# spacemeshos/go-spacemesh

Hardware: AMD Instinct MI355X
Metric: post_labels_per_sec (higher is better)
Workload: dtype u32; 1 GPU; init-mainnet-scryptN8192-4units-256GiB-sink; step_labels=2097152, scrypt_n=8192, num_units=4, labels_per_unit=4294967296, parallelism=index-range shards x1, RCCL nonce min-reduce, vrf_nonce_found=True

## Files before the change

go-spacemesh_amd/csrc/kernel_args.h:

```cpp
#ifndef POST_KERNEL_ARGS_H
#define POST_KERNEL_ARGS_H

#include <hip/hip_runtime.h>

#include "post_common.h"

struct LabelKernelArgs {
  uint32_t commitment_le[8];
  uint64_t start;
  uint64_t count;
  uint32_t scrypt_n;
  uint32_t gap_shift;
  uint32_t out_full;
  uint32_t *scratch;
  uint64_t scratch_lanes;
  uint8_t *out;
  const uint64_t *indices;
  const uint32_t *commit_ids;
  const uint32_t *commitments;
  uint32_t *xbuf;
  uint32_t has_difficulty;
  uint32_t difficulty_be[8];
  PostVrfCandidate *cand;
  unsigned int *cand_count;
  uint32_t cand_cap;
};

struct ScanKernelArgs {
  const uint4 *labels;
  uint64_t count;
  uint64_t index_base;
  const uint32_t *te;
  const uint8_t *sbox;
  const uint32_t *rk;
  uint32_t n_ciphers;
  uint64_t difficulty;
  PostScanHit *hits;
  unsigned int *hit_count;
  uint32_t hit_cap;
};

struct VerifyPredArgs {
  const uint4 *labels2;
  uint64_t count;
  const uint32_t *te;
  const uint8_t *sbox;
  const uint32_t *rk;
  const uint32_t *task_proof;
  const uint8_t *half;
  const uint64_t *difficulty;
  uint8_t *pass;
};

extern "C" {
hipError_t poste_launch_label_kernel(const LabelKernelArgs *args,
                                     uint32_t blocks, hipStream_t stream);
hipError_t poste_launch_verify_pred_kernel(const VerifyPredArgs *args,
                                           uint32_t blocks,
                                           hipStream_t stream);
hipError_t poste_launch_scan_kernel(const ScanKernelArgs *args,
                                    uint32_t blocks, hipStream_t stream);
uint64_t poste_label_resident_slots(uint32_t gap_shift);
}

#endif
```

go-spacemesh_amd/csrc/kernels.hip:

```cpp
#include <hip/hip_runtime.h>

#include <cstdlib>
#include <cstring>

#include "kernel_args.h"
#include "post_common.h"

#define POSTE_THREADS 256

#if defined(POSTE_NT) && POSTE_NT
typedef uint32_t poste_v4u __attribute__((ext_vector_type(4)));
#define VSTORE(p, v)                                                           \
  do {                                                                         \
    uint4 _t = (v);                                                            \
    __builtin_nontemporal_store(*(poste_v4u *)&_t, (poste_v4u *)(p));          \
  } while (0)
#define VLOAD(p)                                                               \
  ({                                                                           \
    poste_v4u _r = __builtin_nontemporal_load((const poste_v4u *)(p));         \
    *(uint4 *)&_r;                                                             \
  })
#else
#define VSTORE(p, v) (*(p) = (v))
#define VLOAD(p) (*(p))
#endif

__constant__ uint32_t c_sha_k[64] = {
    0x428a2f98, 0x71374491, 0xb5c0fbcf, 0xe9b5dba5, 0x3956c25b, 0x59f111f1,
    0x923f82a4, 0xab1c5ed5, 0xd807aa98, 0x12835b01, 0x243185be, 0x550c7dc3,
    0x72be5d74, 0x80deb1fe, 0x9bdc06a7, 0xc19bf174, 0xe49b69c1, 0xefbe4786,
    0x0fc19dc6, 0x240ca1cc, 0x2de92c6f, 0x4a7484aa, 0x5cb0a9dc, 0x76f988da,
    0x983e5152, 0xa831c66d, 0xb00327c8, 0xbf597fc7, 0xc6e00bf3, 0xd5a79147,
    0x06ca6351, 0x14292967, 0x27b70a85, 0x2e1b2138, 0x4d2c6dfc, 0x53380d13,
    0x650a7354, 0x766a0abb, 0x81c2c92e, 0x92722c85, 0xa2bfe8a1, 0xa81a664b,
    0xc24b8b70, 0xc76c51a3, 0xd192e819, 0xd6990624, 0xf40e3585, 0x106aa070,
    0x19a4c116, 0x1e376c08, 0x2748774c, 0x34b0bcb5, 0x391c0cb3, 0x4ed8aa4a,
    0x5b9cca4f, 0x682e6ff3, 0x748f82ee, 0x78a5636f, 0x84c87814, 0x8cc70208,
    0x90befffa, 0xa4506ceb, 0xbef9a3f7, 0xc67178f2};

__device__ __forceinline__ uint32_t ror32(uint32_t x, int n) {
  return __builtin_rotateright32(x, n);
}

__device__ void sha_compress(uint32_t h[8], const uint32_t m[16]) {
  uint32_t w[16];
#pragma unroll
  for (int i = 0; i < 16; i++) w[i] = m[i];
  uint32_t a = h[0], b = h[1], c = h[2], d = h[3];
  uint32_t e = h[4], f = h[5], g = h[6], hh = h[7];
#pragma unroll
  for (int t = 0; t < 64; t++) {
    uint32_t wt;
    if (t < 16) {
      wt = w[t];
    } else {
      uint32_t a15 = w[(t - 15) & 15], a2 = w[(t - 2) & 15];
      wt = w[t & 15] += (ror32(a15, 7) ^ ror32(a15, 18) ^ (a15 >> 3)) +
                        w[(t - 7) & 15] +
                        (ror32(a2, 17) ^ ror32(a2, 19) ^ (a2 >> 10));
    }
    uint32_t t1 = hh + (ror32(e, 6) ^ ror32(e, 11) ^ ror32(e, 25)) +
                  ((e & f) ^ (~e & g)) + c_sha_k[t] + wt;
    uint32_t t2 = (ror32(a, 2) ^ ror32(a, 13) ^ ror32(a, 22)) +
                  ((a & b) ^ (a & c) ^ (b & c));
    hh = g; g = f; f = e; e = d + t1;
    d = c; c = b; b = a; a = t1 + t2;
  }
  h[0] += a; h[1] += b; h[2] += c; h[3] += d;
  h[4] += e; h[5] += f; h[6] += g; h[7] += hh;
}

__device__ __forceinline__ void sha_init(uint32_t h[8]) {
  h[0] = 0x6a09e667; h[1] = 0xbb67ae85; h[2] = 0x3c6ef372; h[3] = 0xa54ff53a;
  h[4] = 0x510e527f; h[5] = 0x9b05688c; h[6] = 0x1f83d9ab; h[7] = 0x5be0cd19;
}


#define SWZ(v, pat)                                                            \
  ((uint32_t)__builtin_amdgcn_mov_dpp((int)(v), (pat), 0xf, 0xf, true))
#define QROT1 0x39
#define QROT2 0x4E
#define QROT3 0x93
#define QBCAST0 0x00

__device__ __forceinline__ void salsa8_z(uint32_t &A, uint32_t &B,
                                         uint32_t &C, uint32_t &D) {
  uint32_t a = A, b = B, c = C, d = D;
#pragma unroll
  for (int i = 0; i < 4; i++) {
    b ^= __builtin_rotateleft32(a + d, 7);
    c ^= __builtin_rotateleft32(b + a, 9);
    d ^= __builtin_rotateleft32(c + b, 13);
    a ^= __builtin_rotateleft32(d + c, 18);
    uint32_t y1 = SWZ(d, QROT1);
    uint32_t y2 = SWZ(c, QROT2);
    uint32_t y3 = SWZ(b, QROT3);
    y1 ^= __builtin_rotateleft32(a + y3, 7);
    y2 ^= __builtin_rotateleft32(y1 + a, 9);
    y3 ^= __builtin_rotateleft32(y2 + y1, 13);
    a ^= __builtin_rotateleft32(y3 + y2, 18);
    d = SWZ(y1, QROT3);
    c = SWZ(y2, QROT2);
    b = SWZ(y3, QROT1);
  }
  A += a; B += b; C += c; D += d;
}

__device__ __forceinline__ void salsa8_z2(uint32_t &A0, uint32_t &B0,
                                          uint32_t &C0, uint32_t &D0,
                                          uint32_t &A1, uint32_t &B1,
                                          uint32_t &C1, uint32_t &D1) {
  uint32_t a0 = A0, b0 = B0, c0 = C0, d0 = D0;
  uint32_t a1 = A1, b1 = B1, c1 = C1, d1 = D1;
#pragma unroll
  for (int i = 0; i < 4; i++) {
    b0 ^= __builtin_rotateleft32(a0 + d0, 7);
    b1 ^= __builtin_rotateleft32(a1 + d1, 7);
    c0 ^= __builtin_rotateleft32(b0 + a0, 9);
    c1 ^= __builtin_rotateleft32(b1 + a1, 9);
    d0 ^= __builtin_rotateleft32(c0 + b0, 13);
    d1 ^= __builtin_rotateleft32(c1 + b1, 13);
    a0 ^= __builtin_rotateleft32(d0 + c0, 18);
    a1 ^= __builtin_rotateleft32(d1 + c1, 18);
    uint32_t y30 = SWZ(b0, QROT3), y31 = SWZ(b1, QROT3);
    uint32_t y20 = SWZ(c0, QROT2), y21 = SWZ(c1, QROT2);
    uint32_t y10 = SWZ(d0, QROT1), y11 = SWZ(d1, QROT1);
    y10 ^= __builtin_rotateleft32(a0 + y30, 7);
    y11 ^= __builtin_rotateleft32(a1 + y31, 7);
    y20 ^= __builtin_rotateleft32(y10 + a0, 9);
    y21 ^= __builtin_rotateleft32(y11 + a1, 9);
    y30 ^= __builtin_rotateleft32(y20 + y10, 13);
    y31 ^= __builtin_rotateleft32(y21 + y11, 13);
    a0 ^= __builtin_rotateleft32(y30 + y20, 18);
    a1 ^= __builtin_rotateleft32(y31 + y21, 18);
    d0 = SWZ(y10, QROT3);
    d1 = SWZ(y11, QROT3);
    c0 = SWZ(y20, QROT2);
    c1 = SWZ(y21, QROT2);
    b0 = SWZ(y30, QROT1);
    b1 = SWZ(y31, QROT1);
  }
  A0 += a0; B0 += b0; C0 += c0; D0 += d0;
  A1 += a1; B1 += b1; C1 += c1; D1 += d1;
}

__device__ __forceinline__ void blockmix2_z(uint32_t XA0[4], uint32_t XA1[4],
                                            uint32_t XB0[4],
                                            uint32_t XB1[4]) {
  uint32_t ta0 = XA0[0] ^ XA1[0], ta1 = XA0[1] ^ XA1[1],
           ta2 = XA0[2] ^ XA1[2], ta3 = XA0[3] ^ XA1[3];
  uint32_t tb0 = XB0[0] ^ XB1[0], tb1 = XB0[1] ^ XB1[1],
           tb2 = XB0[2] ^ XB1[2], tb3 = XB0[3] ^ XB1[3];
  salsa8_z2(ta0, ta1, ta2, ta3, tb0, tb1, tb2, tb3);
  XA0[0] = ta0; XA0[1] = ta1; XA0[2] = ta2; XA0[3] = ta3;
  XB0[0] = tb0; XB0[1] = tb1; XB0[2] = tb2; XB0[3] = tb3;
  ta0 ^= XA1[0]; ta1 ^= XA1[1]; ta2 ^= XA1[2]; ta3 ^= XA1[3];
  tb0 ^= XB1[0]; tb1 ^= XB1[1]; tb2 ^= XB1[2]; tb3 ^= XB1[3];
  salsa8_z2(ta0, ta1, ta2, ta3, tb0, tb1, tb2, tb3);
  XA1[0] = ta0; XA1[1] = ta1; XA1[2] = ta2; XA1[3] = ta3;
  XB1[0] = tb0; XB1[1] = tb1; XB1[2] = tb2; XB1[3] = tb3;
}

__device__ __forceinline__ void blockmix_z(uint32_t X0[4], uint32_t X1[4]) {
  uint32_t t0 = X0[0] ^ X1[0], t1 = X0[1] ^ X1[1], t2 = X0[2] ^ X1[2],
           t3 = X0[3] ^ X1[3];
  salsa8_z(t0, t1, t2, t3);
  X0[0] = t0; X0[1] = t1; X0[2] = t2; X0[3] = t3;
  t0 ^= X1[0]; t1 ^= X1[1]; t2 ^= X1[2]; t3 ^= X1[3];
  salsa8_z(t0, t1, t2, t3);
  X1[0] = t0; X1[1] = t1; X1[2] = t2; X1[3] = t3;
}

__device__ __forceinline__ void canon_to_z(const uint32_t x[16], uint32_t sub,
                                           uint32_t z[4]) {
  uint32_t s0 = sub == 0 ? x[0] : sub == 1 ? x[5] : sub == 2 ? x[10] : x[15];
  uint32_t s1 = sub == 0 ? x[4] : sub == 1 ? x[9] : sub == 2 ? x[14] : x[3];
  uint32_t s2 = sub == 0 ? x[8] : sub == 1 ? x[13] : sub == 2 ? x[2] : x[7];
  uint32_t s3 = sub == 0 ? x[12] : sub == 1 ? x[1] : sub == 2 ? x[6] : x[11];
  z[0] = s0; z[1] = s1; z[2] = s2; z[3] = s3;
}

__device__ __forceinline__ void z_to_msg_be(const uint32_t z[4],
                                            uint32_t m[16]) {
#pragma unroll
  for (int v = 0; v < 4; v++) {
    m[(4 * v + 0) & 15] = __builtin_bswap32(SWZ(z[v], 0x00));
    m[(4 * v + 5) & 15] = __builtin_bswap32(SWZ(z[v], 0x55));
    m[(4 * v + 10) & 15] = __builtin_bswap32(SWZ(z[v], 0xAA));
    m[(4 * v + 15) & 15] = __builtin_bswap32(SWZ(z[v], 0xFF));
  }
}


__device__ __forceinline__ void hmac_outer(const uint32_t ho[8],
                                           const uint32_t inner[8],
                                           uint32_t out[8]) {
  uint32_t h[8], m[16];
#pragma unroll
  for (int i = 0; i < 8; i++) h[i] = ho[i];
#pragma unroll
  for (int i = 0; i < 8; i++) m[i] = inner[i];
  m[8] = 0x80000000u;
#pragma unroll
  for (int i = 9; i < 15; i++) m[i] = 0;
  m[15] = (64 + 32) * 8;
  sha_compress(h, m);
#pragma unroll
  for (int i = 0; i < 8; i++) out[i] = h[i];
}


__device__ __forceinline__ void hmac_states_for(const uint32_t *cw,
                                                unsigned long long index,
                                                uint32_t hi[8],
                                                uint32_t ho[8]) {
  uint32_t pw_be[10], m[16];
#pragma unroll
  for (int i = 0; i < 8; i++) pw_be[i] = __builtin_bswap32(cw[i]);
  pw_be[8] = __builtin_bswap32((uint32_t)index);
  pw_be[9] = __builtin_bswap32((uint32_t)(index >> 32));
  sha_init(hi);
#pragma unroll
  for (int i = 0; i < 10; i++) m[i] = pw_be[i] ^ 0x36363636u;
#pragma unroll
  for (int i = 10; i < 16; i++) m[i] = 0x36363636u;
  sha_compress(hi, m);
  sha_init(ho);
#pragma unroll
  for (int i = 0; i < 10; i++) m[i] = pw_be[i] ^ 0x5c5c5c5cu;
#pragma unroll
  for (int i = 10; i < 16; i++) m[i] = 0x5c5c5c5cu;
  sha_compress(ho, m);
}

__global__ void __launch_bounds__(POSTE_THREADS)
post_label_prologue_kernel(LabelKernelArgs a) {
  const unsigned long long lane =
      (unsigned long long)blockIdx.x * blockDim.x + threadIdx.x;
  const unsigned long long group = lane >> 2;
  const unsigned long long gstride =
      ((unsigned long long)gridDim.x * blockDim.x) >> 2;
  const uint32_t sub = (uint32_t)(lane & 3);
  uint4 *X = (uint4 *)a.xbuf;

  for (unsigned long long task = group; task < a.count;
       task += gstride) {
    const unsigned long long index = a.indices ? a.indices[task]
                                               : a.start + task;
    const uint32_t *cw = a.commit_ids
                             ? a.commitments + 8ull * a.commit_ids[task]
                             : a.commitment_le;
    uint32_t hi[8], ho[8], m[16];
    hmac_states_for(cw, index, hi, ho);
    uint32_t Z0[4], Z1[4];
    for (uint32_t half = 0; half < 2; half++) {
      uint32_t cblk[16];
#pragma unroll
      for (uint32_t q = 0; q < 2; q++) {
        const uint32_t blk = half * 2 + q + 1;
        uint32_t h[8];
#pragma unroll
        for (int i = 0; i < 8; i++) h[i] = hi[i];
        m[0] = blk;
        m[1] = 0x80000000u;
#pragma unroll
        for (int i = 2; i < 15; i++) m[i] = 0;
        m[15] = (64 + 4) * 8;
        sha_compress(h, m);
        uint32_t d[8];
        hmac_outer(ho, h, d);
#pragma unroll
        for (int k = 0; k < 8; k++)
          cblk[8 * q + k] = __builtin_bswap32(d[k]);
      }
      canon_to_z(cblk, sub, half == 0 ? Z0 : Z1);
    }
    uint4 *p = X + task * 8ull;
    p[sub] = make_uint4(Z0[0], Z0[1], Z0[2], Z0[3]);
    p[sub + 4] = make_uint4(Z1[0], Z1[1], Z1[2], Z1[3]);
  }
}

__global__ void __launch_bounds__(POSTE_THREADS, 8)
post_label_romix_kernel(LabelKernelArgs a) {
  const unsigned long long lane =
      (unsigned long long)blockIdx.x * blockDim.x + threadIdx.x;
  const unsigned long long group = lane >> 2;
  const uint32_t sub = (uint32_t)(lane & 3);
  const uint32_t n = a.scrypt_n;
  const uint32_t mask = n - 1;
  const uint32_t gmask = (1u << a.gap_shift) - 1u;
  uint4 *V = (uint4 *)a.scratch;
  uint4 *X = (uint4 *)a.xbuf;

  for (unsigned long long task = group; task < a.count;
       task += a.scratch_lanes) {
    uint32_t Z0[4], Z1[4];
    {
      uint4 *p = X + task * 8ull;
      uint4 v0 = p[sub], v1 = p[sub + 4];
      Z0[0] = v0.x; Z0[1] = v0.y; Z0[2] = v0.z; Z0[3] = v0.w;
      Z1[0] = v1.x; Z1[1] = v1.y; Z1[2] = v1.z; Z1[3] = v1.w;
    }
    {
      unsigned long long base = group * 8ull + sub;
      const unsigned long long stride = a.scratch_lanes * 8ull;
      for (uint32_t j = 0; j < n; j++) {
        if ((j & gmask) == 0) {
          uint4 *p = V + base;
          VSTORE(p, make_uint4(Z0[0], Z0[1], Z0[2], Z0[3]));
          VSTORE(p + 4, make_uint4(Z1[0], Z1[1], Z1[2], Z1[3]));
          base += stride;
        }
        blockmix_z(Z0, Z1);
      }
    }
    for (uint32_t i = 0; i < n; i++) {
      uint32_t j = SWZ(Z1[0], QBCAST0) & mask;
      const uint32_t r = j & gmask;
      const uint4 *p =
          V + ((unsigned long long)(j >> a.gap_shift) * a.scratch_lanes +
               group) * 8ull + sub;
      uint32_t Y0[4], Y1[4];
      {
        uint4 v0 = VLOAD(p), v1 = VLOAD(p + 4);
        Y0[0] = v0.x; Y0[1] = v0.y; Y0[2] = v0.z; Y0[3] = v0.w;
        Y1[0] = v1.x; Y1[1] = v1.y; Y1[2] = v1.z; Y1[3] = v1.w;
      }
      for (uint32_t t = 0; t < r; t++) blockmix_z(Y0, Y1);
#pragma unroll
      for (int k = 0; k < 4; k++) {
        Z0[k] ^= Y0[k];
        Z1[k] ^= Y1[k];
      }
      blockmix_z(Z0, Z1);
    }
    {
      uint4 *p = X + task * 8ull;
      p[sub] = make_uint4(Z0[0], Z0[1], Z0[2], Z0[3]);
      p[sub + 4] = make_uint4(Z1[0], Z1[1], Z1[2], Z1[3]);
    }
  }
}

__global__ void __launch_bounds__(POSTE_THREADS, 8)
post_label_romix2_kernel(LabelKernelArgs a) {
  const unsigned long long lane =
      (unsigned long long)blockIdx.x * blockDim.x + threadIdx.x;
  const unsigned long long group = lane >> 2;
  const uint32_t sub = (uint32_t)(lane & 3);
  const unsigned long long gquads =
      ((unsigned long long)gridDim.x * blockDim.x) >> 2;
  const uint32_t n = a.scrypt_n;
  const uint32_t mask = n - 1;
  uint4 *V = (uint4 *)a.scratch;
  uint4 *X = (uint4 *)a.xbuf;
  const unsigned long long slotA = group * 2, slotB = group * 2 + 1;

  for (unsigned long long base = group * 2; base < a.count;
       base += 2 * gquads) {
    const unsigned long long taskA = base;
    const unsigned long long taskB = base + 1;
    const bool validB = taskB < a.count;
    const unsigned long long tb = validB ? taskB : taskA;
    uint32_t ZA0[4], ZA1[4], ZB0[4], ZB1[4];
    {
      uint4 *pA = X + taskA * 8ull;
      uint4 *pB = X + tb * 8ull;
      uint4 a0 = pA[sub], a1 = pA[sub + 4];
      uint4 b0 = pB[sub], b1 = pB[sub + 4];
      ZA0[0] = a0.x; ZA0[1] = a0.y; ZA0[2] = a0.z; ZA0[3] = a0.w;
      ZA1[0] = a1.x; ZA1[1] = a1.y; ZA1[2] = a1.z; ZA1[3] = a1.w;
      ZB0[0] = b0.x; ZB0[1] = b0.y; ZB0[2] = b0.z; ZB0[3] = b0.w;
      ZB1[0] = b1.x; ZB1[1] = b1.y; ZB1[2] = b1.z; ZB1[3] = b1.w;
    }
    {
      unsigned long long baseA = slotA * 8ull + sub;
      unsigned long long baseB = slotB * 8ull + sub;
      const unsigned long long stride = a.scratch_lanes * 8ull;
      for (uint32_t j = 0; j < n; j++) {
        uint4 *pA = V + baseA;
        uint4 *pB = V + baseB;
        pA[0] = make_uint4(ZA0[0], ZA0[1], ZA0[2], ZA0[3]);
        pA[4] = make_uint4(ZA1[0], ZA1[1], ZA1[2], ZA1[3]);
        pB[0] = make_uint4(ZB0[0], ZB0[1], ZB0[2], ZB0[3]);
        pB[4] = make_uint4(ZB1[0], ZB1[1], ZB1[2], ZB1[3]);
        blockmix2_z(ZA0, ZA1, ZB0, ZB1);
        baseA += stride;
        baseB += stride;
      }
    }
    for (uint32_t i = 0; i < n; i++) {
      uint32_t jA = SWZ(ZA1[0], QBCAST0) & mask;
      uint32_t jB = SWZ(ZB1[0], QBCAST0) & mask;
      const uint4 *pA =
          V + ((unsigned long long)jA * a.scratch_lanes + slotA) * 8ull + sub;
      const uint4 *pB =
          V + ((unsigned long long)jB * a.scratch_lanes + slotB) * 8ull + sub;
      uint4 va0 = pA[0], va1 = pA[4];
      uint4 vb0 = pB[0], vb1 = pB[4];
      ZA0[0] ^= va0.x; ZA0[1] ^= va0.y; ZA0[2] ^= va0.z; ZA0[3] ^= va0.w;
      ZA1[0] ^= va1.x; ZA1[1] ^= va1.y; ZA1[2] ^= va1.z; ZA1[3] ^= va1.w;
      ZB0[0] ^= vb0.x; ZB0[1] ^= vb0.y; ZB0[2] ^= vb0.z; ZB0[3] ^= vb0.w;
      ZB1[0] ^= vb1.x; ZB1[1] ^= vb1.y; ZB1[2] ^= vb1.z; ZB1[3] ^= vb1.w;
      blockmix2_z(ZA0, ZA1, ZB0, ZB1);
    }
    {
      uint4 *pA = X + taskA * 8ull;
      pA[sub] = make_uint4(ZA0[0], ZA0[1], ZA0[2], ZA0[3]);
      pA[sub + 4] = make_uint4(ZA1[0], ZA1[1], ZA1[2], ZA1[3]);
      if (validB) {
        uint4 *pB = X + taskB * 8ull;
        pB[sub] = make_uint4(ZB0[0], ZB0[1], ZB0[2], ZB0[3]);
        pB[sub + 4] = make_uint4(ZB1[0], ZB1[1], ZB1[2], ZB1[3]);
      }
    }
  }
}

__global__ void __launch_bounds__(POSTE_THREADS)
post_label_tail_kernel(LabelKernelArgs a) {
  const unsigned long long lane =
      (unsigned long long)blockIdx.x * blockDim.x + threadIdx.x;
  const unsigned long long group = lane >> 2;
  const unsigned long long gstride =
      ((unsigned long long)gridDim.x * blockDim.x) >> 2;
  const uint32_t sub = (uint32_t)(lane & 3);
  uint4 *X = (uint4 *)a.xbuf;

  uint32_t min_lab[8];
  unsigned long long min_idx = 0;
  int min_found = 0;

  for (unsigned long long task = group; task < a.count;
       task += gstride) {
    const unsigned long long index = a.indices ? a.indices[task]
                                               : a.start + task;
    const uint32_t *cw = a.commit_ids
                             ? a.commitments + 8ull * a.commit_ids[task]
                             : a.commitment_le;
    uint32_t hi[8], ho[8], m[16];
    hmac_states_for(cw, index, hi, ho);
    uint32_t Z0[4], Z1[4];
    {
      uint4 *p = X + task * 8ull;
      uint4 v0 = p[sub], v1 = p[sub + 4];
      Z0[0] = v0.x; Z0[1] = v0.y; Z0[2] = v0.z; Z0[3] = v0.w;
      Z1[0] = v1.x; Z1[1] = v1.y; Z1[2] = v1.z; Z1[3] = v1.w;
    }
    uint32_t h[8];
#pragma unroll
    for (int i = 0; i < 8; i++) h[i] = hi[i];
    z_to_msg_be(Z0, m);
    sha_compress(h, m);
    z_to_msg_be(Z1, m);
    sha_compress(h, m);
    m[0] = 1;
    m[1] = 0x80000000u;
#pragma unroll
    for (int i = 2; i < 15; i++) m[i] = 0;
    m[15] = (64 + 128 + 4) * 8;
    sha_compress(h, m);
    uint32_t lab_be[8];
    hmac_outer(ho, h, lab_be);

    if (a.out && sub == 0) {
      if (a.out_full) {
        uint4 *o = (uint4 *)(a.out + task * 32ull);
        o[0] = make_uint4(__builtin_bswap32(lab_be[0]),
                          __builtin_bswap32(lab_be[1]),
                          __builtin_bswap32(lab_be[2]),
                          __builtin_bswap32(lab_be[3]));
        o[1] = make_uint4(__builtin_bswap32(lab_be[4]),
                          __builtin_bswap32(lab_be[5]),
                          __builtin_bswap32(lab_be[6]),
                          __builtin_bswap32(lab_be[7]));
      } else {
        *(uint4 *)(a.out + task * 16ull) =
            make_uint4(__builtin_bswap32(lab_be[0]),
                       __builtin_bswap32(lab_be[1]),
                       __builtin_bswap32(lab_be[2]),
                       __builtin_bswap32(lab_be[3]));
      }
    }

    if (a.has_difficulty && sub == 0) {
      bool below_diff = false, below_min = false;
#pragma unroll
      for (int k = 0; k < 8; k++) {
        if (lab_be[k] != a.difficulty_be[k]) {
          below_diff = lab_be[k] < a.difficulty_be[k];
          break;
        }
      }
      if (below_diff) {
        if (!min_found) {
          below_min = true;
        } else {
          below_min = false;
#pragma unroll
          for (int k = 0; k < 8; k++) {
            if (lab_be[k] != min_lab[k]) {
              below_min = lab_be[k] < min_lab[k];
              break;
            }
          }
        }
        if (below_min) {
          min_found = 1;
          min_idx = index;
#pragma unroll
          for (int k = 0; k < 8; k++) min_lab[k] = lab_be[k];
        }
      }
    }
  }

  if (a.has_difficulty) {
    __shared__ uint32_t s_lab[POSTE_THREADS][8];
    __shared__ unsigned long long s_idx[POSTE_THREADS];
    __shared__ uint8_t s_found[POSTE_THREADS];
    s_found[threadIdx.x] = (uint8_t)min_found;
    if (min_found) {
      s_idx[threadIdx.x] = min_idx;
#pragma unroll
      for (int k = 0; k < 8; k++) s_lab[threadIdx.x][k] = min_lab[k];
    }
    __syncthreads();
    if (threadIdx.x == 0) {
      int best = -1;
      for (int t = 0; t < POSTE_THREADS; t++) {
        if (!s_found[t]) continue;
        if (best < 0) {
          best = t;
          continue;
        }
        int cmp = 0;
        for (int k = 0; k < 8 && cmp == 0; k++) {
          if (s_lab[t][k] < s_lab[best][k]) cmp = -1;
          else if (s_lab[t][k] > s_lab[best][k]) cmp = 1;
        }
        if (cmp < 0 || (cmp == 0 && s_idx[t] < s_idx[best])) best = t;
      }
      if (best >= 0) {
        unsigned int slot = atomicAdd(a.cand_count, 1u);
        if (slot < a.cand_cap) {
          a.cand[slot].index = s_idx[best];
          for (int k = 0; k < 8; k++)
            a.cand[slot].label_be[k] = s_lab[best][k];
        }
      }
    }
  }
}


__global__ void __launch_bounds__(POSTE_THREADS)
post_scan_kernel(ScanKernelArgs a) {
#if defined(POSTE_SCAN_GLOBAL_TT)
  const uint32_t *TE_LO = a.te;
  const uint32_t *TE_HI = a.te;
  const uint8_t *sSbox = a.sbox;
#elif defined(POSTE_SCAN_SPLIT_TT)
  extern __shared__ uint32_t lds[];
  uint32_t *TE_LO = lds;
  const uint32_t *TE_HI = a.te;
  uint8_t *sSbox = (uint8_t *)(lds + 512);
  for (uint32_t i = threadIdx.x; i < 512; i += blockDim.x) TE_LO[i] = a.te[i];
  for (uint32_t i = threadIdx.x; i < 256; i += blockDim.x)
    sSbox[i] = a.sbox[i];
  __syncthreads();
#else
  extern __shared__ uint32_t lds[];
  uint32_t *sTe = lds;
  uint8_t *sSbox = (uint8_t *)(sTe + 1024);
  uint32_t *TE_LO = sTe, *TE_HI = sTe;

  for (uint32_t i = threadIdx.x; i < 1024; i += blockDim.x) sTe[i] = a.te[i];
  for (uint32_t i = threadIdx.x; i < 256; i += blockDim.x)
    sSbox[i] = a.sbox[i];
  __syncthreads();
#endif

  const unsigned long long stride =
      (unsigned long long)gridDim.x * blockDim.x;
#ifndef POSTE_SCAN_ILP
#define POSTE_SCAN_ILP 2
#endif
  constexpr int L = POSTE_SCAN_ILP;
  const unsigned long long span = stride * L;
  for (unsigned long long t0 =
           (unsigned long long)blockIdx.x * blockDim.x + threadIdx.x;
       t0 < a.count; t0 += span) {
    uint32_t p[L][4];
    unsigned long long ts[L];
#pragma unroll
    for (int u = 0; u < L; u++) {
      unsigned long long t = t0 + (unsigned long long)u * stride;
      ts[u] = t < a.count ? t : t0;
      uint4 lraw = a.labels[ts[u]];
      p[u][0] = __builtin_bswap32(lraw.x);
      p[u][1] = __builtin_bswap32(lraw.y);
      p[u][2] = __builtin_bswap32(lraw.z);
      p[u][3] = __builtin_bswap32(lraw.w);
    }
    const int live = (int)((a.count - t0 + stride - 1) / stride) < L
                         ? (int)((a.count - t0 + stride - 1) / stride)
                         : L;
    for (uint32_t c = 0; c < a.n_ciphers; c++) {
      const uint32_t *rk = a.rk + c * 44;
      uint32_t w[L][4];
#pragma unroll
      for (int u = 0; u < L; u++)
#pragma unroll
        for (int k = 0; k < 4; k++) w[u][k] = p[u][k] ^ rk[k];
#pragma unroll
      for (int r = 1; r < 10; r++) {
#pragma unroll
        for (int u = 0; u < L; u++) {
          uint32_t n0 = TE_LO[w[u][0] >> 24] ^
                        TE_LO[256 + ((w[u][1] >> 16) & 0xff)] ^
                        TE_HI[512 + ((w[u][2] >> 8) & 0xff)] ^
                        TE_HI[768 + (w[u][3] & 0xff)] ^ rk[4 * r];
          uint32_t n1 = TE_LO[w[u][1] >> 24] ^
                        TE_LO[256 + ((w[u][2] >> 16) & 0xff)] ^
                        TE_HI[512 + ((w[u][3] >> 8) & 0xff)] ^
                        TE_HI[768 + (w[u][0] & 0xff)] ^ rk[4 * r + 1];
          uint32_t n2 = TE_LO[w[u][2] >> 24] ^
                        TE_LO[256 + ((w[u][3] >> 16) & 0xff)] ^
                        TE_HI[512 + ((w[u][0] >> 8) & 0xff)] ^
                        TE_HI[768 + (w[u][1] & 0xff)] ^ rk[4 * r + 2];
          uint32_t n3 = TE_LO[w[u][3] >> 24] ^
                        TE_LO[256 + ((w[u][0] >> 16) & 0xff)] ^
                        TE_HI[512 + ((w[u][1] >> 8) & 0xff)] ^
                        TE_HI[768 + (w[u][2] & 0xff)] ^ rk[4 * r + 3];
          w[u][0] = n0; w[u][1] = n1; w[u][2] = n2; w[u][3] = n3;
        }
      }
#pragma unroll
      for (int u = 0; u < L; u++) {
        if (u >= live) break;
        uint32_t f0 = (((uint32_t)sSbox[w[u][0] >> 24] << 24) |
                       ((uint32_t)sSbox[(w[u][1] >> 16) & 0xff] << 16) |
                       ((uint32_t)sSbox[(w[u][2] >> 8) & 0xff] << 8) |
                       sSbox[w[u][3] & 0xff]) ^ rk[40];
        uint32_t f1 = (((uint32_t)sSbox[w[u][1] >> 24] << 24) |
                       ((uint32_t)sSbox[(w[u][2] >> 16) & 0xff] << 16) |
                       ((uint32_t)sSbox[(w[u][3] >> 8) & 0xff] << 8) |
                       sSbox[w[u][0] & 0xff]) ^ rk[41];
        uint32_t f2 = (((uint32_t)sSbox[w[u][2] >> 24] << 24) |
                       ((uint32_t)sSbox[(w[u][3] >> 16) & 0xff] << 16) |
                       ((uint32_t)sSbox[(w[u][0] >> 8) & 0xff] << 8) |
                       sSbox[w[u][1] & 0xff]) ^ rk[42];
        uint32_t f3 = (((uint32_t)sSbox[w[u][3] >> 24] << 24) |
                       ((uint32_t)sSbox[(w[u][0] >> 16) & 0xff] << 16) |
                       ((uint32_t)sSbox[(w[u][1] >> 8) & 0xff] << 8) |
                       sSbox[w[u][2] & 0xff]) ^ rk[43];
        unsigned long long v0 =
            __builtin_bswap64(((unsigned long long)f0 << 32) | f1);
        unsigned long long v1 =
            __builtin_bswap64(((unsigned long long)f2 << 32) | f3);
        if (v0 < a.difficulty) {
          unsigned int s = atomicAdd(a.hit_count, 1u);
          if (s < a.hit_cap) {
            a.hits[s].index = a.index_base + ts[u];
            a.hits[s].nonce = c * POSTE_NONCES_PER_AES;
          }
        }
        if (v1 < a.difficulty) {
          unsigned int s = atomicAdd(a.hit_count, 1u);
          if (s < a.hit_cap) {
            a.hits[s].index = a.index_base + ts[u];
            a.hits[s].nonce = c * POSTE_NONCES_PER_AES + 1;
          }
        }
      }
    }
  }
}

#define ROR8(x) __builtin_amdgcn_alignbit((x), (x), 8)
#define ROR16(x) __builtin_amdgcn_alignbit((x), (x), 16)
#define ROR24(x) __builtin_amdgcn_alignbit((x), (x), 24)

template <int THREADS_, bool BATCHG>
__global__ void __launch_bounds__(THREADS_)
post_scan_bankrep_kernel(ScanKernelArgs a) {
  extern __shared__ uint32_t sTe[];
  for (uint32_t i = threadIdx.x; i < 8192; i += blockDim.x)
    sTe[i] = a.te[i >> 5];
  __syncthreads();
  const uint32_t lane31 = threadIdx.x & 31;
#define TE0R(idx) sTe[(((uint32_t)(idx)) << 5) | lane31]

  const unsigned long long stride =
      (unsigned long long)gridDim.x * blockDim.x;
#ifndef POSTE_SCAN_ILP
#define POSTE_SCAN_ILP 2
#endif
  constexpr int L = POSTE_SCAN_ILP;
  const unsigned long long span = stride * L;
  for (unsigned long long t0 =
           (unsigned long long)blockIdx.x * blockDim.x + threadIdx.x;
       t0 < a.count; t0 += span) {
    uint32_t p[L][4];
    unsigned long long ts[L];
#pragma unroll
    for (int u = 0; u < L; u++) {
      unsigned long long t = t0 + (unsigned long long)u * stride;
      ts[u] = t < a.count ? t : t0;
      uint4 lraw = a.labels[ts[u]];
      p[u][0] = __builtin_bswap32(lraw.x);
      p[u][1] = __builtin_bswap32(lraw.y);
      p[u][2] = __builtin_bswap32(lraw.z);
      p[u][3] = __builtin_bswap32(lraw.w);
    }
    const int live = (int)((a.count - t0 + stride - 1) / stride) < L
                         ? (int)((a.count - t0 + stride - 1) / stride)
                         : L;
    for (uint32_t c = 0; c < a.n_ciphers; c++) {
      uint32_t rk[44];
#pragma unroll
      for (int k = 0; k < 44; k++) rk[k] = a.rk[c * 44 + k];
      uint32_t w[L][4];
#pragma unroll
      for (int u = 0; u < L; u++)
#pragma unroll
        for (int k = 0; k < 4; k++) w[u][k] = p[u][k] ^ rk[k];
#pragma unroll
      for (int r = 1; r < 10; r++) {
        if (BATCHG) {
          uint32_t g[L][16];
#pragma unroll
          for (int u = 0; u < L; u++)
#pragma unroll
            for (int q = 0; q < 4; q++) {
              g[u][4 * q + 0] = TE0R(w[u][q] >> 24);
              g[u][4 * q + 1] = TE0R((w[u][(q + 1) & 3] >> 16) & 0xff);
              g[u][4 * q + 2] = TE0R((w[u][(q + 2) & 3] >> 8) & 0xff);
              g[u][4 * q + 3] = TE0R(w[u][(q + 3) & 3] & 0xff);
            }
#pragma unroll
          for (int u = 0; u < L; u++)
#pragma unroll
            for (int q = 0; q < 4; q++)
              w[u][q] = g[u][4 * q] ^ ROR8(g[u][4 * q + 1]) ^
                        ROR16(g[u][4 * q + 2]) ^ ROR24(g[u][4 * q + 3]) ^
                        rk[4 * r + q];
        } else {
#pragma unroll
        for (int u = 0; u < L; u++) {
          uint32_t n0 = TE0R(w[u][0] >> 24) ^
                        ROR8(TE0R((w[u][1] >> 16) & 0xff)) ^
                        ROR16(TE0R((w[u][2] >> 8) & 0xff)) ^
                        ROR24(TE0R(w[u][3] & 0xff)) ^ rk[4 * r];
          uint32_t n1 = TE0R(w[u][1] >> 24) ^
                        ROR8(TE0R((w[u][2] >> 16) & 0xff)) ^
                        ROR16(TE0R((w[u][3] >> 8) & 0xff)) ^
                        ROR24(TE0R(w[u][0] & 0xff)) ^ rk[4 * r + 1];
          uint32_t n2 = TE0R(w[u][2] >> 24) ^
                        ROR8(TE0R((w[u][3] >> 16) & 0xff)) ^
                        ROR16(TE0R((w[u][0] >> 8) & 0xff)) ^
                        ROR24(TE0R(w[u][1] & 0xff)) ^ rk[4 * r + 2];
          uint32_t n3 = TE0R(w[u][3] >> 24) ^
                        ROR8(TE0R((w[u][0] >> 16) & 0xff)) ^
                        ROR16(TE0R((w[u][1] >> 8) & 0xff)) ^
                        ROR24(TE0R(w[u][2] & 0xff)) ^ rk[4 * r + 3];
          w[u][0] = n0; w[u][1] = n1; w[u][2] = n2; w[u][3] = n3;
        }
        }
      }
#define SB24(idx) ((TE0R(idx) & 0xff00u) << 16)
#define SB16(idx) ((TE0R(idx) & 0xff00u) << 8)
#define SB08(idx) (TE0R(idx) & 0xff00u)
#define SB00(idx) ((TE0R(idx) >> 8) & 0xffu)
#pragma unroll
      for (int u = 0; u < L; u++) {
        if (u >= live) break;
        uint32_t f0 = (SB24(w[u][0] >> 24) | SB16((w[u][1] >> 16) & 0xff) |
                       SB08((w[u][2] >> 8) & 0xff) | SB00(w[u][3] & 0xff)) ^
                      rk[40];
        uint32_t f1 = (SB24(w[u][1] >> 24) | SB16((w[u][2] >> 16) & 0xff) |
                       SB08((w[u][3] >> 8) & 0xff) | SB00(w[u][0] & 0xff)) ^
                      rk[41];
        uint32_t f2 = (SB24(w[u][2] >> 24) | SB16((w[u][3] >> 16) & 0xff) |
                       SB08((w[u][0] >> 8) & 0xff) | SB00(w[u][1] & 0xff)) ^
                      rk[42];
        uint32_t f3 = (SB24(w[u][3] >> 24) | SB16((w[u][0] >> 16) & 0xff) |
                       SB08((w[u][1] >> 8) & 0xff) | SB00(w[u][2] & 0xff)) ^
                      rk[43];
        unsigned long long v0 =
            __builtin_bswap64(((unsigned long long)f0 << 32) | f1);
        unsigned long long v1 =
            __builtin_bswap64(((unsigned long long)f2 << 32) | f3);
        if (v0 < a.difficulty) {
          unsigned int s = atomicAdd(a.hit_count, 1u);
          if (s < a.hit_cap) {
            a.hits[s].index = a.index_base + ts[u];
            a.hits[s].nonce = c * POSTE_NONCES_PER_AES;
          }
        }
        if (v1 < a.difficulty) {
          unsigned int s = atomicAdd(a.hit_count, 1u);
          if (s < a.hit_cap) {
            a.hits[s].index = a.index_base + ts[u];
            a.hits[s].nonce = c * POSTE_NONCES_PER_AES + 1;
          }
        }
      }
    }
  }
#undef TE0R
#undef SB24
#undef SB16
#undef SB08
#undef SB00
}

__global__ void __launch_bounds__(1024)
post_scan_tt4_kernel(ScanKernelArgs a) {
  extern __shared__ uint32_t sTe[];
  for (uint32_t i = threadIdx.x; i < 32768; i += blockDim.x)
    sTe[i] = a.te[((i >> 5) & 3) * 256 + (i >> 7)];
  __syncthreads();
  const uint32_t *t0p = sTe + (threadIdx.x & 31);
#define TT4(t, idx) t0p[(((uint32_t)(idx)) << 7) + 32 * (t)]

  const unsigned long long stride =
      (unsigned long long)gridDim.x * blockDim.x;
  constexpr int L = POSTE_SCAN_ILP > 4 ? POSTE_SCAN_ILP : 4;
  const unsigned long long span = stride * L;
  for (unsigned long long t0 =
           (unsigned long long)blockIdx.x * blockDim.x + threadIdx.x;
       t0 < a.count; t0 += span) {
    uint32_t p[L][4];
    unsigned long long ts[L];
#pragma unroll
    for (int u = 0; u < L; u++) {
      unsigned long long t = t0 + (unsigned long long)u * stride;
      ts[u] = t < a.count ? t : t0;
      uint4 lraw = a.labels[ts[u]];
      p[u][0] = __builtin_bswap32(lraw.x);
      p[u][1] = __builtin_bswap32(lraw.y);
      p[u][2] = __builtin_bswap32(lraw.z);
      p[u][3] = __builtin_bswap32(lraw.w);
    }
    const int live = (int)((a.count - t0 + stride - 1) / stride) < L
                         ? (int)((a.count - t0 + stride - 1) / stride)
                         : L;
    for (uint32_t c = 0; c < a.n_ciphers; c++) {
      uint32_t rk[44];
#pragma unroll
      for (int k = 0; k < 44; k++) rk[k] = a.rk[c * 44 + k];
      uint32_t w[L][4];
#pragma unroll
      for (int u = 0; u < L; u++)
#pragma unroll
        for (int k = 0; k < 4; k++) w[u][k] = p[u][k] ^ rk[k];
#pragma unroll
      for (int r = 1; r < 10; r++) {
#pragma unroll
        for (int u = 0; u < L; u++) {
          uint32_t n0 = TT4(0, w[u][0] >> 24) ^
                        TT4(1, (w[u][1] >> 16) & 0xff) ^
                        TT4(2, (w[u][2] >> 8) & 0xff) ^
                        TT4(3, w[u][3] & 0xff) ^ rk[4 * r];
          uint32_t n1 = TT4(0, w[u][1] >> 24) ^
                        TT4(1, (w[u][2] >> 16) & 0xff) ^
                        TT4(2, (w[u][3] >> 8) & 0xff) ^
                        TT4(3, w[u][0] & 0xff) ^ rk[4 * r + 1];
          uint32_t n2 = TT4(0, w[u][2] >> 24) ^
                        TT4(1, (w[u][3] >> 16) & 0xff) ^
                        TT4(2, (w[u][0] >> 8) & 0xff) ^
                        TT4(3, w[u][1] & 0xff) ^ rk[4 * r + 2];
          uint32_t n3 = TT4(0, w[u][3] >> 24) ^
                        TT4(1, (w[u][0] >> 16) & 0xff) ^
                        TT4(2, (w[u][1] >> 8) & 0xff) ^
                        TT4(3, w[u][2] & 0xff) ^ rk[4 * r + 3];
          w[u][0] = n0; w[u][1] = n1; w[u][2] = n2; w[u][3] = n3;
        }
      }
#define SB24_4(idx) ((TT4(0, idx) & 0xff00u) << 16)
#define SB16_4(idx) ((TT4(0, idx) & 0xff00u) << 8)
#define SB08_4(idx) (TT4(0, idx) & 0xff00u)
#define SB00_4(idx) ((TT4(0, idx) >> 8) & 0xffu)
#pragma unroll
      for (int u = 0; u < L; u++) {
        if (u >= live) break;
        uint32_t f0 = (SB24_4(w[u][0] >> 24) |
                       SB16_4((w[u][1] >> 16) & 0xff) |
                       SB08_4((w[u][2] >> 8) & 0xff) |
                       SB00_4(w[u][3] & 0xff)) ^ rk[40];
        uint32_t f1 = (SB24_4(w[u][1] >> 24) |
                       SB16_4((w[u][2] >> 16) & 0xff) |
                       SB08_4((w[u][3] >> 8) & 0xff) |
                       SB00_4(w[u][0] & 0xff)) ^ rk[41];
        uint32_t f2 = (SB24_4(w[u][2] >> 24) |
                       SB16_4((w[u][3] >> 16) & 0xff) |
                       SB08_4((w[u][0] >> 8) & 0xff) |
                       SB00_4(w[u][1] & 0xff)) ^ rk[42];
        uint32_t f3 = (SB24_4(w[u][3] >> 24) |
                       SB16_4((w[u][0] >> 16) & 0xff) |
                       SB08_4((w[u][1] >> 8) & 0xff) |
                       SB00_4(w[u][2] & 0xff)) ^ rk[43];
        unsigned long long v0 =
            __builtin_bswap64(((unsigned long long)f0 << 32) | f1);
        unsigned long long v1 =
            __builtin_bswap64(((unsigned long long)f2 << 32) | f3);
        if (v0 < a.difficulty) {
          unsigned int s = atomicAdd(a.hit_count, 1u);
          if (s < a.hit_cap) {
            a.hits[s].index = a.index_base + ts[u];
            a.hits[s].nonce = c * POSTE_NONCES_PER_AES;
          }
        }
        if (v1 < a.difficulty) {
          unsigned int s = atomicAdd(a.hit_count, 1u);
          if (s < a.hit_cap) {
            a.hits[s].index = a.index_base + ts[u];
            a.hits[s].nonce = c * POSTE_NONCES_PER_AES + 1;
          }
        }
      }
    }
  }
#undef TT4
#undef SB24_4
#undef SB16_4
#undef SB08_4
#undef SB00_4
}

__global__ void __launch_bounds__(POSTE_THREADS)
post_verify_pred_kernel(VerifyPredArgs a) {
  extern __shared__ uint32_t lds[];
  uint32_t *sTe = lds;
  uint8_t *sSbox = (uint8_t *)(sTe + 1024);
  for (uint32_t i = threadIdx.x; i < 1024; i += blockDim.x) sTe[i] = a.te[i];
  for (uint32_t i = threadIdx.x; i < 256; i += blockDim.x)
    sSbox[i] = a.sbox[i];
  __syncthreads();
  const unsigned long long stride =
      (unsigned long long)gridDim.x * blockDim.x;
  for (unsigned long long t =
           (unsigned long long)blockIdx.x * blockDim.x + threadIdx.x;
       t < a.count; t += stride) {
    const uint32_t pidx = a.task_proof[t];
    const uint32_t *rk = a.rk + (unsigned long long)pidx * 44;
    uint4 lraw = a.labels2[2 * t];
    uint32_t w0 = __builtin_bswap32(lraw.x) ^ rk[0];
    uint32_t w1 = __builtin_bswap32(lraw.y) ^ rk[1];
    uint32_t w2 = __builtin_bswap32(lraw.z) ^ rk[2];
    uint32_t w3 = __builtin_bswap32(lraw.w) ^ rk[3];
#pragma unroll
    for (int r = 1; r < 10; r++) {
      uint32_t n0 = sTe[w0 >> 24] ^ sTe[256 + ((w1 >> 16) & 0xff)] ^
                    sTe[512 + ((w2 >> 8) & 0xff)] ^ sTe[768 + (w3 & 0xff)] ^
                    rk[4 * r];
      uint32_t n1 = sTe[w1 >> 24] ^ sTe[256 + ((w2 >> 16) & 0xff)] ^
                    sTe[512 + ((w3 >> 8) & 0xff)] ^ sTe[768 + (w0 & 0xff)] ^
                    rk[4 * r + 1];
      uint32_t n2 = sTe[w2 >> 24] ^ sTe[256 + ((w3 >> 16) & 0xff)] ^
                    sTe[512 + ((w0 >> 8) & 0xff)] ^ sTe[768 + (w1 & 0xff)] ^
                    rk[4 * r + 2];
      uint32_t n3 = sTe[w3 >> 24] ^ sTe[256 + ((w0 >> 16) & 0xff)] ^
                    sTe[512 + ((w1 >> 8) & 0xff)] ^ sTe[768 + (w2 & 0xff)] ^
                    rk[4 * r + 3];
      w0 = n0; w1 = n1; w2 = n2; w3 = n3;
    }
    uint32_t f0 = (((uint32_t)sSbox[w0 >> 24] << 24) |
                   ((uint32_t)sSbox[(w1 >> 16) & 0xff] << 16) |
                   ((uint32_t)sSbox[(w2 >> 8) & 0xff] << 8) |
                   sSbox[w3 & 0xff]) ^ rk[40];
    uint32_t f1 = (((uint32_t)sSbox[w1 >> 24] << 24) |
                   ((uint32_t)sSbox[(w2 >> 16) & 0xff] << 16) |
                   ((uint32_t)sSbox[(w3 >> 8) & 0xff] << 8) |
                   sSbox[w0 & 0xff]) ^ rk[41];
    uint32_t f2 = (((uint32_t)sSbox[w2 >> 24] << 24) |
                   ((uint32_t)sSbox[(w3 >> 16) & 0xff] << 16) |
                   ((uint32_t)sSbox[(w0 >> 8) & 0xff] << 8) |
                   sSbox[w1 & 0xff]) ^ rk[42];
    uint32_t f3 = (((uint32_t)sSbox[w3 >> 24] << 24) |
                   ((uint32_t)sSbox[(w0 >> 16) & 0xff] << 16) |
                   ((uint32_t)sSbox[(w1 >> 8) & 0xff] << 8) |
                   sSbox[w2 & 0xff]) ^ rk[43];
    unsigned long long v =
        a.half[pidx] == 0
            ? __builtin_bswap64(((unsigned long long)f0 << 32) | f1)
            : __builtin_bswap64(((unsigned long long)f2 << 32) | f3);
    a.pass[t] = v < a.difficulty[pidx] ? 1 : 0;
  }
}

extern "C" {

hipError_t poste_launch_label_kernel(const LabelKernelArgs *args,
                                     uint32_t blocks, hipStream_t stream) {
  static const bool use2 = [] {
    const char *e = getenv("POST_ROMIX2");
    return e && e[0] == '1';
  }();
  const bool dual = use2 && args->gap_shift == 0;
  uint32_t gblocks = dual ? (blocks + 1) / 2 : blocks;
  hipLaunchKernelGGL(post_label_prologue_kernel, dim3(gblocks),
                     dim3(POSTE_THREADS), 0, stream, *args);
  if (dual) {
    hipLaunchKernelGGL(post_label_romix2_kernel, dim3(gblocks),
                       dim3(POSTE_THREADS), 0, stream, *args);
  } else {
    hipLaunchKernelGGL(post_label_romix_kernel, dim3(blocks),
                       dim3(POSTE_THREADS), 0, stream, *args);
  }
  hipLaunchKernelGGL(post_label_tail_kernel, dim3(gblocks),
                     dim3(POSTE_THREADS), 0, stream, *args);
  return hipGetLastError();
}

hipError_t poste_launch_verify_pred_kernel(const VerifyPredArgs *args,
                                           uint32_t blocks,
                                           hipStream_t stream) {
  size_t lds = 1024 * 4 + 256;
  hipLaunchKernelGGL(post_verify_pred_kernel, dim3(blocks),
                     dim3(POSTE_THREADS), lds, stream, *args);
  return hipGetLastError();
}

uint64_t poste_label_resident_slots(uint32_t gap_shift) {
  const void *kern =
      gap_shift == 0
          ? reinterpret_cast<const void *>(post_label_romix2_kernel)
          : reinterpret_cast<const void *>(post_label_romix_kernel);
  int blocks_per_cu = 0;
  if (hipOccupancyMaxActiveBlocksPerMultiprocessor(&blocks_per_cu, kern,
                                                   POSTE_THREADS, 0) !=
          hipSuccess ||
      blocks_per_cu <= 0)
    blocks_per_cu = 2;
  hipDeviceProp_t prop;
  int dev = 0;
  (void)hipGetDevice(&dev);
  int cus = 256;
  if (hipGetDeviceProperties(&prop, dev) == hipSuccess)
    cus = prop.multiProcessorCount;
  uint64_t quads = (uint64_t)blocks_per_cu * cus * (POSTE_THREADS / 4);
  const char *e = getenv("POST_ROMIX2");
  const bool dual = e && e[0] == '1' && gap_shift == 0;
  return dual ? quads * 2 : quads;
}

hipError_t poste_launch_scan_kernel(const ScanKernelArgs *args,
                                    uint32_t blocks, hipStream_t stream) {
  const char *e = getenv("POST_SCAN_MODE");
  const char *m = e ? e : "tt4";
  if (strcmp(m, "shared") == 0) {
    size_t lds = 1024 * 4 + 256;
    hipLaunchKernelGGL(post_scan_kernel, dim3(blocks), dim3(POSTE_THREADS),
                       lds, stream, *args);
    return hipGetLastError();
  }
  if (strcmp(m, "tt4") == 0) {
    static bool attr_ok = [] {
      return hipFuncSetAttribute(
                 (const void *)post_scan_tt4_kernel,
                 hipFuncAttributeMaxDynamicSharedMemorySize,
                 32768 * 4) == hipSuccess;
    }();
    if (attr_ok) {
      uint32_t b4 = (uint32_t)((args->count + 1023) / 1024);
      if (b4 > 2048) b4 = 2048;
      if (b4 == 0) b4 = 1;
      hipLaunchKernelGGL(post_scan_tt4_kernel, dim3(b4), dim3(1024),
                         32768 * 4, stream, *args);
      return hipGetLastError();
    }
    m = "bankrep";
  }
  const bool bg = strstr(m, "bg") != nullptr;
  const bool wide = strstr(m, "512") != nullptr;
  size_t lds = 8192 * 4;
  if (wide) {
    uint32_t b5 = (uint32_t)((args->count + 511) / 512);
    if (b5 > 4096) b5 = 4096;
    if (b5 == 0) b5 = 1;
    if (bg)
      hipLaunchKernelGGL((post_scan_bankrep_kernel<512, true>), dim3(b5),
                         dim3(512), lds, stream, *args);
    else
      hipLaunchKernelGGL((post_scan_bankrep_kernel<512, false>), dim3(b5),
                         dim3(512), lds, stream, *args);
  } else if (bg) {
    hipLaunchKernelGGL((post_scan_bankrep_kernel<POSTE_THREADS, true>),
                       dim3(blocks), dim3(POSTE_THREADS), lds, stream,
                       *args);
  } else {
    hipLaunchKernelGGL((post_scan_bankrep_kernel<POSTE_THREADS, false>),
                       dim3(blocks), dim3(POSTE_THREADS), lds, stream,
                       *args);
  }
  return hipGetLastError();
}
}
```

Before: 2.038 million labels/s.

## Add lean single-task ROMix kernel with 24-bit indexing and fused XOR3

Replaces the opt-in dual-task ROMix kernel with a lean single-task kernel that runs by default when gap_shift is zero and the sizes fit. It uses a precomputed per-quad base pointer with a 24-bit masked stride so scratch address math stays in 32-bit multiplies. It also uses optional nontemporal loads and stores for the V buffer and folds the V XOR into blockmix with a three-input bitop3. The old gap kernel is kept as the fallback, and the dual-task ILP path is removed.

```diff
diff --git a/go-spacemesh_amd/csrc/kernel_args.h b/go-spacemesh_amd/csrc/kernel_args.h
--- a/go-spacemesh_amd/csrc/kernel_args.h
+++ b/go-spacemesh_amd/csrc/kernel_args.h
@@ -61,6 +61,8 @@
 hipError_t poste_launch_scan_kernel(const ScanKernelArgs *args,
                                     uint32_t blocks, hipStream_t stream);
 uint64_t poste_label_resident_slots(uint32_t gap_shift);
+int poste_label_romix_lean_ok(uint32_t scrypt_n, uint32_t gap_shift,
+                              uint64_t scratch_lanes);
 }
 
 #endif
diff --git a/go-spacemesh_amd/csrc/kernels.hip b/go-spacemesh_amd/csrc/kernels.hip
--- a/go-spacemesh_amd/csrc/kernels.hip
+++ b/go-spacemesh_amd/csrc/kernels.hip
@@ -106,61 +106,6 @@
   A += a; B += b; C += c; D += d;
 }
 
-__device__ __forceinline__ void salsa8_z2(uint32_t &A0, uint32_t &B0,
-                                          uint32_t &C0, uint32_t &D0,
-                                          uint32_t &A1, uint32_t &B1,
-                                          uint32_t &C1, uint32_t &D1) {
-  uint32_t a0 = A0, b0 = B0, c0 = C0, d0 = D0;
-  uint32_t a1 = A1, b1 = B1, c1 = C1, d1 = D1;
-#pragma unroll
-  for (int i = 0; i < 4; i++) {
-    b0 ^= __builtin_rotateleft32(a0 + d0, 7);
-    b1 ^= __builtin_rotateleft32(a1 + d1, 7);
-    c0 ^= __builtin_rotateleft32(b0 + a0, 9);
-    c1 ^= __builtin_rotateleft32(b1 + a1, 9);
-    d0 ^= __builtin_rotateleft32(c0 + b0, 13);
-    d1 ^= __builtin_rotateleft32(c1 + b1, 13);
-    a0 ^= __builtin_rotateleft32(d0 + c0, 18);
-    a1 ^= __builtin_rotateleft32(d1 + c1, 18);
-    uint32_t y30 = SWZ(b0, QROT3), y31 = SWZ(b1, QROT3);
-    uint32_t y20 = SWZ(c0, QROT2), y21 = SWZ(c1, QROT2);
-    uint32_t y10 = SWZ(d0, QROT1), y11 = SWZ(d1, QROT1);
-    y10 ^= __builtin_rotateleft32(a0 + y30, 7);
-    y11 ^= __builtin_rotateleft32(a1 + y31, 7);
-    y20 ^= __builtin_rotateleft32(y10 + a0, 9);
-    y21 ^= __builtin_rotateleft32(y11 + a1, 9);
-    y30 ^= __builtin_rotateleft32(y20 + y10, 13);
-    y31 ^= __builtin_rotateleft32(y21 + y11, 13);
-    a0 ^= __builtin_rotateleft32(y30 + y20, 18);
-    a1 ^= __builtin_rotateleft32(y31 + y21, 18);
-    d0 = SWZ(y10, QROT3);
-    d1 = SWZ(y11, QROT3);
-    c0 = SWZ(y20, QROT2);
-    c1 = SWZ(y21, QROT2);
-    b0 = SWZ(y30, QROT1);
-    b1 = SWZ(y31, QROT1);
-  }
-  A0 += a0; B0 += b0; C0 += c0; D0 += d0;
-  A1 += a1; B1 += b1; C1 += c1; D1 += d1;
-}
-
-__device__ __forceinline__ void blockmix2_z(uint32_t XA0[4], uint32_t XA1[4],
-                                            uint32_t XB0[4],
-                                            uint32_t XB1[4]) {
-  uint32_t ta0 = XA0[0] ^ XA1[0], ta1 = XA0[1] ^ XA1[1],
-           ta2 = XA0[2] ^ XA1[2], ta3 = XA0[3] ^ XA1[3];
-  uint32_t tb0 = XB0[0] ^ XB1[0], tb1 = XB0[1] ^ XB1[1],
-           tb2 = XB0[2] ^ XB1[2], tb3 = XB0[3] ^ XB1[3];
-  salsa8_z2(ta0, ta1, ta2, ta3, tb0, tb1, tb2, tb3);
-  XA0[0] = ta0; XA0[1] = ta1; XA0[2] = ta2; XA0[3] = ta3;
-  XB0[0] = tb0; XB0[1] = tb1; XB0[2] = tb2; XB0[3] = tb3;
-  ta0 ^= XA1[0]; ta1 ^= XA1[1]; ta2 ^= XA1[2]; ta3 ^= XA1[3];
-  tb0 ^= XB1[0]; tb1 ^= XB1[1]; tb2 ^= XB1[2]; tb3 ^= XB1[3];
-  salsa8_z2(ta0, ta1, ta2, ta3, tb0, tb1, tb2, tb3);
-  XA1[0] = ta0; XA1[1] = ta1; XA1[2] = ta2; XA1[3] = ta3;
-  XB1[0] = tb0; XB1[1] = tb1; XB1[2] = tb2; XB1[3] = tb3;
-}
-
 __device__ __forceinline__ void blockmix_z(uint32_t X0[4], uint32_t X1[4]) {
   uint32_t t0 = X0[0] ^ X1[0], t1 = X0[1] ^ X1[1], t2 = X0[2] ^ X1[2],
            t3 = X0[3] ^ X1[3];
@@ -282,7 +227,7 @@
 }
 
 __global__ void __launch_bounds__(POSTE_THREADS, 8)
-post_label_romix_kernel(LabelKernelArgs a) {
+post_label_romix_gap_kernel(LabelKernelArgs a) {
   const unsigned long long lane =
       (unsigned long long)blockIdx.x * blockDim.x + threadIdx.x;
   const unsigned long long group = lane >> 2;
@@ -343,77 +288,68 @@
   }
 }
 
+#define POSTE_U24 0xffffffu
+
+__device__ __forceinline__ const uint4 *vblock(const uint4 *qbase, uint32_t j,
+                                               uint32_t stride16) {
+  return qbase + (unsigned long long)j * stride16;
+}
+
+#define XOR3(a, b, c) ((uint32_t)__builtin_amdgcn_bitop3_b32((a), (b), (c), 0x96))
+
+__device__ __forceinline__ void blockmix_xor_z(uint32_t X0[4], uint32_t X1[4],
+                                               const uint4 v0,
+                                               const uint4 v1) {
+  X1[0] ^= v1.x; X1[1] ^= v1.y; X1[2] ^= v1.z; X1[3] ^= v1.w;
+  uint32_t t0 = XOR3(X0[0], v0.x, X1[0]), t1 = XOR3(X0[1], v0.y, X1[1]),
+           t2 = XOR3(X0[2], v0.z, X1[2]), t3 = XOR3(X0[3], v0.w, X1[3]);
+  salsa8_z(t0, t1, t2, t3);
+  X0[0] = t0; X0[1] = t1; X0[2] = t2; X0[3] = t3;
+  t0 ^= X1[0]; t1 ^= X1[1]; t2 ^= X1[2]; t3 ^= X1[3];
+  salsa8_z(t0, t1, t2, t3);
+  X1[0] = t0; X1[1] = t1; X1[2] = t2; X1[3] = t3;
+}
+
 __global__ void __launch_bounds__(POSTE_THREADS, 8)
-post_label_romix2_kernel(LabelKernelArgs a) {
+post_label_romix_kernel(LabelKernelArgs a) {
   const unsigned long long lane =
       (unsigned long long)blockIdx.x * blockDim.x + threadIdx.x;
   const unsigned long long group = lane >> 2;
   const uint32_t sub = (uint32_t)(lane & 3);
-  const unsigned long long gquads =
-      ((unsigned long long)gridDim.x * blockDim.x) >> 2;
   const uint32_t n = a.scrypt_n;
-  const uint32_t mask = n - 1;
-  uint4 *V = (uint4 *)a.scratch;
+  const uint32_t mask = (n - 1) & POSTE_U24;
+  const uint32_t stride16 = ((uint32_t)a.scratch_lanes * 8u) & POSTE_U24;
+  uint4 *const qbase = (uint4 *)a.scratch + (group * 8ull + sub);
   uint4 *X = (uint4 *)a.xbuf;
-  const unsigned long long slotA = group * 2, slotB = group * 2 + 1;
-
-  for (unsigned long long base = group * 2; base < a.count;
-       base += 2 * gquads) {
-    const unsigned long long taskA = base;
-    const unsigned long long taskB = base + 1;
-    const bool validB = taskB < a.count;
-    const unsigned long long tb = validB ? taskB : taskA;
-    uint32_t ZA0[4], ZA1[4], ZB0[4], ZB1[4];
+
+  for (unsigned long long task = group; task < a.count;
+       task += a.scratch_lanes) {
+    uint32_t Z0[4], Z1[4];
     {
-      uint4 *pA = X + taskA * 8ull;
-      uint4 *pB = X + tb * 8ull;
-      uint4 a0 = pA[sub], a1 = pA[sub + 4];
-      uint4 b0 = pB[sub], b1 = pB[sub + 4];
-      ZA0[0] = a0.x; ZA0[1] = a0.y; ZA0[2] = a0.z; ZA0[3] = a0.w;
-      ZA1[0] = a1.x; ZA1[1] = a1.y; ZA1[2] = a1.z; ZA1[3] = a1.w;
-      ZB0[0] = b0.x; ZB0[1] = b0.y; ZB0[2] = b0.z; ZB0[3] = b0.w;
-      ZB1[0] = b1.x; ZB1[1] = b1.y; ZB1[2] = b1.z; ZB1[3] = b1.w;
+      uint4 *p = X + task * 8ull;
+      uint4 v0 = p[sub], v1 = p[sub + 4];
+      Z0[0] = v0.x; Z0[1] = v0.y; Z0[2] = v0.z; Z0[3] = v0.w;
+      Z1[0] = v1.x; Z1[1] = v1.y; Z1[2] = v1.z; Z1[3] = v1.w;
     }
     {
-      unsigned long long baseA = slotA * 8ull + sub;
-      unsigned long long baseB = slotB * 8ull + sub;
-      const unsigned long long stride = a.scratch_lanes * 8ull;
+      uint4 *p = qbase;
       for (uint32_t j = 0; j < n; j++) {
-        uint4 *pA = V + baseA;
-        uint4 *pB = V + baseB;
-        pA[0] = make_uint4(ZA0[0], ZA0[1], ZA0[2], ZA0[3]);
-        pA[4] = make_uint4(ZA1[0], ZA1[1], ZA1[2], ZA1[3]);
-        pB[0] = make_uint4(ZB0[0], ZB0[1], ZB0[2], ZB0[3]);
-        pB[4] = make_uint4(ZB1[0], ZB1[1], ZB1[2], ZB1[3]);
-        blockmix2_z(ZA0, ZA1, ZB0, ZB1);
-        baseA += stride;
-        baseB += stride;
+        VSTORE(p, make_uint4(Z0[0], Z0[1], Z0[2], Z0[3]));
+        VSTORE(p + 4, make_uint4(Z1[0], Z1[1], Z1[2], Z1[3]));
+        p += stride16;
+        blockmix_z(Z0, Z1);
       }
     }
     for (uint32_t i = 0; i < n; i++) {
-      uint32_t jA = SWZ(ZA1[0], QBCAST0) & mask;
-      uint32_t jB = SWZ(ZB1[0], QBCAST0) & mask;
-      const uint4 *pA =
-          V + ((unsigned long long)jA * a.scratch_lanes + slotA) * 8ull + sub;
-      const uint4 *pB =
-          V + ((unsigned long long)jB * a.scratch_lanes + slotB) * 8ull + sub;
-      uint4 va0 = pA[0], va1 = pA[4];
-      uint4 vb0 = pB[0], vb1 = pB[4];
-      ZA0[0] ^= va0.x; ZA0[1] ^= va0.y; ZA0[2] ^= va0.z; ZA0[3] ^= va0.w;
-      ZA1[0] ^= va1.x; ZA1[1] ^= va1.y; ZA1[2] ^= va1.z; ZA1[3] ^= va1.w;
-      ZB0[0] ^= vb0.x; ZB0[1] ^= vb0.y; ZB0[2] ^= vb0.z; ZB0[3] ^= vb0.w;
-      ZB1[0] ^= vb1.x; ZB1[1] ^= vb1.y; ZB1[2] ^= vb1.z; ZB1[3] ^= vb1.w;
-      blockmix2_z(ZA0, ZA1, ZB0, ZB1);
+      const uint32_t j = SWZ(Z1[0], QBCAST0) & mask;
+      const uint4 *p = vblock(qbase, j, stride16);
+      const uint4 v0 = VLOAD(p), v1 = VLOAD(p + 4);
+      blockmix_xor_z(Z0, Z1, v0, v1);
     }
     {
-      uint4 *pA = X + taskA * 8ull;
-      pA[sub] = make_uint4(ZA0[0], ZA0[1], ZA0[2], ZA0[3]);
-      pA[sub + 4] = make_uint4(ZA1[0], ZA1[1], ZA1[2], ZA1[3]);
-      if (validB) {
-        uint4 *pB = X + taskB * 8ull;
-        pB[sub] = make_uint4(ZB0[0], ZB0[1], ZB0[2], ZB0[3]);
-        pB[sub + 4] = make_uint4(ZB1[0], ZB1[1], ZB1[2], ZB1[3]);
-      }
+      uint4 *p = X + task * 8ull;
+      p[sub] = make_uint4(Z0[0], Z0[1], Z0[2], Z0[3]);
+      p[sub + 4] = make_uint4(Z1[0], Z1[1], Z1[2], Z1[3]);
     }
   }
 }
@@ -994,24 +930,26 @@
 
 extern "C" {
 
+int poste_label_romix_lean_ok(uint32_t scrypt_n, uint32_t gap_shift,
+                              uint64_t scratch_lanes) {
+  return gap_shift == 0 && scrypt_n <= (1u << 24) &&
+         scratch_lanes < (1ull << 21) &&
+         (uint64_t)scrypt_n * scratch_lanes < (1ull << 32);
+}
+
 hipError_t poste_launch_label_kernel(const LabelKernelArgs *args,
                                      uint32_t blocks, hipStream_t stream) {
-  static const bool use2 = [] {
-    const char *e = getenv("POST_ROMIX2");
-    return e && e[0] == '1';
-  }();
-  const bool dual = use2 && args->gap_shift == 0;
-  uint32_t gblocks = dual ? (blocks + 1) / 2 : blocks;
-  hipLaunchKernelGGL(post_label_prologue_kernel, dim3(gblocks),
+  hipLaunchKernelGGL(post_label_prologue_kernel, dim3(blocks),
                      dim3(POSTE_THREADS), 0, stream, *args);
-  if (dual) {
-    hipLaunchKernelGGL(post_label_romix2_kernel, dim3(gblocks),
+  if (poste_label_romix_lean_ok(args->scrypt_n, args->gap_shift,
+                                args->scratch_lanes)) {
+    hipLaunchKernelGGL(post_label_romix_kernel, dim3(blocks),
                        dim3(POSTE_THREADS), 0, stream, *args);
   } else {
-    hipLaunchKernelGGL(post_label_romix_kernel, dim3(blocks),
+    hipLaunchKernelGGL(post_label_romix_gap_kernel, dim3(blocks),
                        dim3(POSTE_THREADS), 0, stream, *args);
   }
-  hipLaunchKernelGGL(post_label_tail_kernel, dim3(gblocks),
+  hipLaunchKernelGGL(post_label_tail_kernel, dim3(blocks),
                      dim3(POSTE_THREADS), 0, stream, *args);
   return hipGetLastError();
 }
@@ -1028,8 +966,8 @@
 uint64_t poste_label_resident_slots(uint32_t gap_shift) {
   const void *kern =
       gap_shift == 0
-          ? reinterpret_cast<const void *>(post_label_romix2_kernel)
-          : reinterpret_cast<const void *>(post_label_romix_kernel);
+          ? reinterpret_cast<const void *>(post_label_romix_kernel)
+          : reinterpret_cast<const void *>(post_label_romix_gap_kernel);
   int blocks_per_cu = 0;
   if (hipOccupancyMaxActiveBlocksPerMultiprocessor(&blocks_per_cu, kern,
                                                    POSTE_THREADS, 0) !=
@@ -1042,10 +980,7 @@
   int cus = 256;
   if (hipGetDeviceProperties(&prop, dev) == hipSuccess)
     cus = prop.multiProcessorCount;
-  uint64_t quads = (uint64_t)blocks_per_cu * cus * (POSTE_THREADS / 4);
-  const char *e = getenv("POST_ROMIX2");
-  const bool dual = e && e[0] == '1' && gap_shift == 0;
-  return dual ? quads * 2 : quads;
+  return (uint64_t)blocks_per_cu * cus * (POSTE_THREADS / 4);
 }
 
 hipError_t poste_launch_scan_kernel(const ScanKernelArgs *args,
```

After: 2.068 million labels/s (median of 6 runs). +1.5%, better.
